# kimerein/sabatinilab-glm

Measured on AMD Instinct MI355X. Metric: IRLS iters/sec on 1M×2000 design mat; CV-grid wall-clock (5-fold×20 λ), lower is better.
Workload: dtype bf16 Hessian (w rounded to bf16, X exact 0/1) / exact-f32 gradient (3 bf16 pieces, f64 slab sums) / f64 coefficients and line search

## Files before the change

### sabatinilab-glm_amd/csrc/lagw.hip

```cpp
#include <algorithm>
#include <cstring>
#include <functional>
#include <map>
#include <mutex>
#include <queue>
#include <type_traits>
#include <vector>

#include "common.h"

namespace sglm {
namespace {

__device__ __forceinline__ int lag_col2(int layout, int m, int K, int b, int ev) {
    return layout ? ev * K + b : b * m + ev;
}

constexpr int kLwRed = 128;

__global__ void __launch_bounds__(256) lag_gram_w_part(const float* __restrict__ W, int64_t ld,
                                                       int32_t n, const int32_t* __restrict__ fits,
                                                       float* __restrict__ part) {
    const float* w = W + (int64_t)fits[blockIdx.y] * ld;
    const int64_t chunk = ((int64_t)n + kLwRed - 1) / kLwRed;
    const int64_t t0 = (int64_t)blockIdx.x * chunk, t1 = min((int64_t)n, t0 + chunk);
    float s = 0.0f;
    for (int64_t t = t0 + threadIdx.x; t < t1; t += 256) s += (float)(__bf16)w[t];
    __shared__ float red[256];
    red[threadIdx.x] = s;
    __syncthreads();
    for (int o = 128; o > 0; o >>= 1) {
        if (threadIdx.x < o) red[threadIdx.x] += red[threadIdx.x + o];
        __syncthreads();
    }
    if (threadIdx.x == 0) part[blockIdx.y * kLwRed + blockIdx.x] = red[0];
}

__global__ void __launch_bounds__(256) lag_gram_w_aux(const float* __restrict__ part,
                                                      const int32_t* __restrict__ fits,
                                                      float* __restrict__ H, int32_t P,
                                                      int32_t p) {
    float* Hf = H + (int64_t)fits[blockIdx.y] * P * P;
    if (blockIdx.x == 0) {
        if (threadIdx.x == 0) {
            float t = 0.0f;
            for (int b = 0; b < kLwRed; ++b) t += part[blockIdx.y * kLwRed + b];
            Hf[(int64_t)p * P + p] = t;
        }
        return;
    }
    const int w = P - p - 1;
    const int64_t tot = (int64_t)P * w;
    for (int64_t e = (int64_t)(blockIdx.x - 1) * 256 + threadIdx.x; e < tot;
         e += (int64_t)(gridDim.x - 1) * 256) {
        const int64_t i = e / w, j = p + 1 + e % w;
        if (i <= j) Hf[i * P + j] = 0.0f;
    }
}

__global__ void __launch_bounds__(256) lag_gram_w_prep(const float* __restrict__ W, int64_t ld,
                                                       int32_t n, const int32_t* __restrict__ fits,
                                                       int32_t nf, int32_t row0, int32_t smin,
                                                       int64_t wlen, int64_t zrow,
                                                       uint16_t* __restrict__ Wt) {
    const int c = blockIdx.y;
    for (int64_t j = (int64_t)blockIdx.x * 256 + threadIdx.x; j < wlen;
         j += (int64_t)gridDim.x * 256) {
        const int64_t i = j + c;
        const int64_t u = i / nf;
        const int f = (int)(i % nf);
        const int64_t t = u - row0 + smin;
        const float x = (t >= 0 && t < n && u < zrow) ? W[(int64_t)fits[f] * ld + t] : 0.0f;
        Wt[c * wlen + j] = __builtin_bit_cast(uint16_t, (__bf16)x);
    }
}

constexpr int kKS2 = 128;
constexpr int kKP2 = kKS2 / 2;
constexpr int kRX2 = kKP2 + 4;
constexpr int kRS2 = 4 * kRX2 + 4;
constexpr int kSentR = -(1 << 28);
constexpr uint32_t kSentW = 0xfffff000u;

typedef short s16x4 __attribute__((ext_vector_type(4)));
typedef __attribute__((address_space(3))) s16x4 lds_s16x4;

struct LagW2Args {
    const uint16_t* Wt;
    int64_t wlen;
    const uint64_t* R;
    const int32_t* occ;
    const int32_t* ev_off;
    const int32_t* bidx;
    const int32_t* fits;
    float* H;
    float* Hb;
    int32_t nf, P, p, m, K, smin, smax, layout, nraw, D, Gm, Gy;
    int32_t njobs;
    int32_t ms;
    int32_t wsh;
    uint16_t jobs[256];
#ifdef SGLM_LAGW_TRACE
    uint64_t* trace;
#endif
};

template <int NCH>
__device__ __forceinline__ int lagw_swz(int row) {
    return NCH == 16 ? ((row & 3) << 2) : (((row >> 1) & 1) << 2);
}

template <int MT, int NT, int WM, int WN, int NH>
struct LagW2Smem {
    static constexpr int MB = WM * MT, NN = WN * NT * 32, ND = MB / NH;
    uint32_t rw[2][ND * kRS2];
    __attribute__((aligned(16))) uint16_t ws[2][kKS2 * NN];
    int32_t vo[4][kKS2];
    uint32_t wo[4][kKS2];
};

template <int MT, int NT, int WM, int WN, int NH>
__global__ void __launch_bounds__(64 * WM * WN) __attribute__((amdgpu_waves_per_eu(2, 2)))
lag_gram_w2_kernel(LagW2Args a) {
    using SM = LagW2Smem<MT, NT, WM, WN, NH>;
    constexpr int NTH = 64 * WM * WN, MB = SM::MB, NN = SM::NN, ND = SM::ND, NCH = NN / 8;
    static_assert(MB % NH == 0, "d rows per piece");
    static_assert((kKS2 * NCH) % NTH == 0, "weight tasks per thread");
    constexpr int kWT = kKS2 * NCH / NTH;
    static_assert((kKP2 * ND) % NTH == 0, "row-word tasks per thread");
    constexpr int kRT = kKP2 * ND / NTH;
    static_assert(kWT <= 4, "staging pieces per K-step");
    __shared__ SM sm;
#ifdef SGLM_LAGW_TRACE
    const uint64_t t_beg = __builtin_amdgcn_s_memrealtime();
#endif
    const int blk = blockIdx.x;
    const int a1 = blk % a.ms;
    if (a1 >= a.m) return;
    int type, half = 0;
    if (a.njobs > 0) {
        if (blk >= a.njobs * a.ms) return;
        const int jb = a.jobs[blk / a.ms];
        type = jb & 0x3fff;
        half = jb >> 14;
    } else {
        type = blk / a.ms;
        if (type >= a.Gm * a.Gy) return;
    }
    const int g = type % a.Gm, y = type / a.Gm;
    const int Tm = a.D * NH;
    const int t0 = g * MB;
    if (t0 >= Tm) return;
    const int di0 = t0 / NH;
    const int n0 = y * NN + a.wsh * di0 * a.nf;
    if (n0 / a.nf >= a.K || min(a.K - 1, (n0 + NN - 1) / a.nf) < di0) return;
    int o_beg = a.ev_off[a1], o_end = a.ev_off[a1 + 1];
    if (half) {
        const int hs = ((o_end - o_beg + kKS2 - 1) / kKS2 + 1) / 2;
        if (half == 1) o_end = min(o_end, o_beg + hs * kKS2);
        else o_beg += hs * kKS2;
    }
    const int nst = max(0, (o_end - o_beg + kKS2 - 1) / kKS2);
    const int tid = threadIdx.x, lane = tid & 63, wave = tid >> 6, h = lane >> 5, r = lane & 31;
    const int wm = wave % WM, wn = wave / WM;

    const __amdgpu_buffer_rsrc_t rsR =
        __builtin_amdgcn_make_buffer_rsrc((void*)a.R, 0, a.nraw * 8, 0x00020000);
    const __amdgpu_buffer_rsrc_t rsW =
        __builtin_amdgcn_make_buffer_rsrc((void*)a.Wt, 0, (int)(uint32_t)(a.wlen * 16), 0x00020000);
    const __amdgpu_buffer_rsrc_t rsO =
        __builtin_amdgcn_make_buffer_rsrc((void*)a.occ, 0, a.ev_off[a.m] * 4, 0x00020000);

    int wk[kWT], wsl[kWT];
#pragma unroll
    for (int i = 0; i < kWT; ++i) {
        const int t = tid + NTH * i;
        wk[i] = t / NCH;
        const int ch = t % NCH;
        wsl[i] = wk[i] * NN + 8 * (ch ^ lagw_swz<NCH>(wk[i]));
        wk[i] = wk[i] | (ch << 16);
    }
    int rkp[kRT], rdl[kRT];
#pragma unroll
    for (int i = 0; i < kRT; ++i) {
        const int t = tid + NTH * i;
        rkp[i] = t / ND;
        rdl[i] = t % ND;
    }

    u32x4 wA[kWT];
    u32x2 rA[kRT][2];
    int32_t oreg = 0;
    bool ovalid = false;

    auto occ_load = [&](int s) __attribute__((always_inline)) {
        const int o = o_beg + s * kKS2 + (tid & (kKS2 - 1));
        ovalid = o < o_end;
        oreg = __builtin_amdgcn_raw_buffer_load_b32(rsO, o * 4, 0, 0);
    };
    auto occ_store = [&](int s) __attribute__((always_inline)) {
        if (tid < kKS2) {
            const int v = ovalid ? oreg : kSentR;
            const int64_t x = (int64_t)(ovalid ? oreg : 0) * a.nf + n0;
            const int c = (int)(x & 7);
            sm.vo[s & 3][tid] = v;
            sm.wo[s & 3][tid] = ovalid ? (uint32_t)(2 * (c * a.wlen + x - c)) : kSentW;
        }
    };
    auto load_w = [&](int s, int i) __attribute__((always_inline)) {
        const uint32_t off = sm.wo[s & 3][wk[i] & 0xffff];
        wA[i] = __builtin_bit_cast(u32x4, __builtin_amdgcn_raw_buffer_load_b128(
                                              rsW, off + 16 * (wk[i] >> 16), 0, 0));
    };
    auto load_r = [&](int s) __attribute__((always_inline)) {
#pragma unroll
        for (int i = 0; i < kRT; ++i)
#pragma unroll
            for (int j = 0; j < 2; ++j) {
                const int u = sm.vo[s & 3][2 * rkp[i] + j] + di0 + rdl[i];
                rA[i][j] = __builtin_bit_cast(
                    u32x2, __builtin_amdgcn_raw_buffer_load_b64(rsR, (uint32_t)u << 3, 0, 0));
            }
    };
    auto store_w = [&](int buf, int i) __attribute__((always_inline)) {
        *reinterpret_cast<u32x4*>(&sm.ws[buf][wsl[i]]) = wA[i];
    };
    auto store_r = [&](int buf) __attribute__((always_inline)) {
#pragma unroll
        for (int i = 0; i < kRT; ++i) {
            uint32_t* dst = &sm.rw[buf][rdl[i] * kRS2 + rkp[i]];
#pragma unroll
            for (int pl = 0; pl < NH; ++pl) {
                const uint32_t w0 = rA[i][0][pl], w1 = rA[i][1][pl];
                dst[(2 * pl) * kRX2] = __builtin_amdgcn_perm(w1, w0, 0x05040100u);
                dst[(2 * pl + 1) * kRX2] = __builtin_amdgcn_perm(w1, w0, 0x07060302u);
            }
        }
    };
    auto data_load = [&](int s) __attribute__((always_inline)) {
#pragma unroll
        for (int i = 0; i < kWT; ++i) load_w(s, i);
        load_r(s);
    };
    auto data_store = [&](int buf) __attribute__((always_inline)) {
#pragma unroll
        for (int i = 0; i < kWT; ++i) store_w(buf, i);
        store_r(buf);
    };

    f32x16 acc[MT][NT];
#pragma unroll
    for (int i = 0; i < MT; ++i)
#pragma unroll
        for (int j = 0; j < NT; ++j) acc[i][j] = (f32x16){};

    int aoff[MT];
    int dmin_w = 1 << 30;
#pragma unroll
    for (int i = 0; i < MT; ++i) {
        const int tau = min(t0 + wm * MT + i, Tm - 1);
        const int dl = tau / NH - di0, hf = tau % NH;
        aoff[i] = dl * kRS2 + (2 * hf + (r >> 4)) * kRX2 + 4 * h;
        if (t0 + wm * MT + i < Tm) dmin_w = min(dmin_w, di0 + dl);
    }
    int j0 = NT, j1 = -1;
#pragma unroll
    for (int j = 0; j < NT; ++j) {
        const int c0 = n0 + (wn * NT + j) * 32;
        const int sb_lo = c0 / a.nf, sb_hi = min(a.K - 1, (c0 + 31) / a.nf);
        if (sb_lo < a.K && sb_hi >= dmin_w) {
            j0 = min(j0, j);
            j1 = max(j1, j);
        }
    }
    const int jcode = __builtin_amdgcn_readfirstlane(j0 > j1 ? -1 : j0 * NT + j1);
    int boff[NT];
    {
        const int g4 = lane >> 4, q = (lane >> 2) & 3, pp = lane & 3;
        const int row = 8 * (g4 >> 1) + q;
#pragma unroll
        for (int j = 0; j < NT; ++j) {
            const int col = (wn * NT + j) * 32 + 16 * (g4 & 1) + 4 * pp;
            boff[j] = row * NN * 2 + 16 * ((col >> 3) ^ lagw_swz<NCH>(row)) + 8 * (pp & 1);
        }
    }
    const uint32_t rsh = (uint32_t)(r - 14 - 16 * (r >> 4)) & 31u;

    auto compute = [&](int s, auto J0c, auto J1c) __attribute__((always_inline)) {
        constexpr int J0 = decltype(J0c)::value, J1 = decltype(J1c)::value;
        const int buf = s & 1;
        const uint32_t* rwb = &sm.rw[buf][0];
        const char* wsb = reinterpret_cast<const char*>(&sm.ws[buf][0]);
        auto fetch = [&](int ks, u32x4 (&wq)[MT], s16x4 (&t1)[NT], s16x4 (&t2)[NT])
                         __attribute__((always_inline)) {
#pragma unroll
            for (int j = J0; j <= J1; ++j) {
                const char* pb = wsb + boff[j] + ks * 16 * NN * 2;
                t1[j] = __builtin_amdgcn_ds_read_tr16_b64_v4i16(
                    (lds_s16x4*)(__attribute__((address_space(3))) char*)pb);
                t2[j] = __builtin_amdgcn_ds_read_tr16_b64_v4i16(
                    (lds_s16x4*)(__attribute__((address_space(3))) char*)(pb + 4 * NN * 2));
            }
#pragma unroll
            for (int i = 0; i < MT; ++i)
                wq[i] = *reinterpret_cast<const u32x4*>(rwb + aoff[i] + 8 * ks);
        };
        auto mult = [&](const u32x4 (&wq)[MT], const s16x4 (&t1)[NT], const s16x4 (&t2)[NT])
                        __attribute__((always_inline)) {
            bf16x8 bq[NT];
#pragma unroll
            for (int j = J0; j <= J1; ++j) {
                const uint2 u1 = __builtin_bit_cast(uint2, t1[j]);
                const uint2 u2 = __builtin_bit_cast(uint2, t2[j]);
                bq[j] = __builtin_bit_cast(bf16x8, make_uint4(u1.x, u1.y, u2.x, u2.y));
            }
            bf16x8 aq[MT];
#pragma unroll
            for (int i = 0; i < MT; ++i) {
                uint32_t dq[4];
#pragma unroll
                for (int q = 0; q < 4; ++q) dq[q] = rotr32(wq[i][q], rsh) & 0x40004000u;
                aq[i] = __builtin_bit_cast(bf16x8, make_uint4(dq[0], dq[1], dq[2], dq[3]));
            }
#pragma unroll
            for (int i = 0; i < MT; ++i)
#pragma unroll
                for (int j = J0; j <= J1; ++j)
                    acc[i][j] = __builtin_amdgcn_mfma_f32_32x32x16_bf16(aq[i], bq[j], acc[i][j],
                                                                        0, 0, 0);
        };
        auto staging = [&](int ks) __attribute__((always_inline)) {
            if (ks < kWT) store_w(buf ^ 1, ks);
            if (ks == kWT) store_r(buf ^ 1);
            if (ks == 4) occ_load(s + 4);
            if (ks >= 4 && ks - 4 < kWT) load_w(s + 2, ks - 4);
            if (ks == 7) load_r(s + 2);
        };
        u32x4 wq[2][MT];
        s16x4 t1[2][NT], t2[2][NT];
        fetch(0, wq[0], t1[0], t2[0]);
#pragma unroll
        for (int ks = 0; ks < kKS2 / 16; ++ks) {
            staging(ks);
            if (ks + 1 < kKS2 / 16)
                fetch(ks + 1, wq[(ks + 1) & 1], t1[(ks + 1) & 1], t2[(ks + 1) & 1]);
            __builtin_amdgcn_sched_barrier(0);
            mult(wq[ks & 1], t1[ks & 1], t2[ks & 1]);
            __builtin_amdgcn_sched_barrier(0);
        }
    };
    auto main_loop = [&](auto J0c, auto J1c) __attribute__((always_inline)) {
#pragma unroll
        for (int j = 0; j < 3; ++j) {
            occ_load(j);
            occ_store(j);
        }
        __syncthreads();
        data_load(0);
        data_store(0);
        occ_load(3);
        data_load(1);
        for (int s = 0; s < nst; ++s) {
            occ_store(s + 3);
            __syncthreads();
            compute(s, J0c, J1c);
        }
    };
    using I0 = std::integral_constant<int, 0>;
    using I1 = std::integral_constant<int, 1>;
    using I2 = std::integral_constant<int, 2>;
    using I3 = std::integral_constant<int, 3>;
    using IN = std::integral_constant<int, -1>;
    if (nst > 0) {
        if constexpr (NT == 4) {
            switch (jcode) {
                case 0: main_loop(I0{}, I0{}); break;
                case 1: main_loop(I0{}, I1{}); break;
                case 2: main_loop(I0{}, I2{}); break;
                case 3: main_loop(I0{}, I3{}); break;
                case 5: main_loop(I1{}, I1{}); break;
                case 6: main_loop(I1{}, I2{}); break;
                case 7: main_loop(I1{}, I3{}); break;
                case 10: main_loop(I2{}, I2{}); break;
                case 11: main_loop(I2{}, I3{}); break;
                case 15: main_loop(I3{}, I3{}); break;
                default: main_loop(I0{}, IN{}); break;
            }
        } else {
            static_assert(NT == 2, "N tiles per wave");
            switch (jcode) {
                case 0: main_loop(I0{}, I0{}); break;
                case 1: main_loop(I0{}, I1{}); break;
                case 3: main_loop(I1{}, I1{}); break;
                default: main_loop(I0{}, IN{}); break;
            }
        }
    }

#pragma unroll
    for (int j = 0; j < NT; ++j) {
        const int nn = n0 + (wn * NT + j) * 32 + r;
        const int sb = nn / a.nf, f = nn % a.nf;
        if (sb >= a.K) continue;
        const int b1 = a.bidx[sb];
        if (b1 < 0) continue;
        float* Hrow = (half == 2 ? a.Hb + (int64_t)f * a.P * a.P
                                 : a.H + (int64_t)a.fits[f] * a.P * a.P) +
                      (int64_t)lag_col2(a.layout, a.m, a.K, b1, a1) * a.P;
#pragma unroll
        for (int i = 0; i < MT; ++i) {
            const int tau = t0 + wm * MT + i;
            if (tau >= Tm) continue;
            const int dd = tau / NH;
            const int hf = tau % NH;
            if (sb < dd) continue;
            const int b2 = a.bidx[sb - dd];
            if (b2 < 0) continue;
#pragma unroll
            for (int q = 0; q < 16; ++q) {
                const int a2 = 32 * hf + (q & 3) + 8 * (q >> 2) + 4 * h;
                const float val = 0.5f * acc[i][j][q];
                if (a2 < a.m) {
                    if (dd == 0 && a2 < a1) continue;
                    Hrow[lag_col2(a.layout, a.m, a.K, b2, a2)] = val;
                } else if (a2 == a.m && dd == 0) {
                    Hrow[a.p] = val;
                }
            }
        }
    }
#ifdef SGLM_LAGW_TRACE
    __syncthreads();
    if (tid == 0) {
        const uint64_t t_end = __builtin_amdgcn_s_memrealtime();
        const uint32_t hw = __builtin_amdgcn_s_getreg(4 | (31 << 11));
        const uint32_t xcc = __builtin_amdgcn_s_getreg(20 | (31 << 11));
        a.trace[4 * blk + 0] = t_beg;
        a.trace[4 * blk + 1] = t_end;
        a.trace[4 * blk + 2] = (uint64_t)hw | ((uint64_t)xcc << 32);
        a.trace[4 * blk + 3] = (uint64_t)type | ((uint64_t)a1 << 16) | ((uint64_t)nst << 32);
    }
#endif
}

struct LagwSplit {
    const float* Hb;
    int32_t smin, nh, MB, NN, Gm, nf, wsh;
    uint32_t mask[8];
};

__global__ void __launch_bounds__(256) lag_gram_w_sym(float* __restrict__ H,
                                                      const int32_t* __restrict__ fits, int32_t P,
                                                      int32_t p, int32_t m, int32_t K,
                                                      int32_t layout,
                                                      const int32_t* __restrict__ shifts,
                                                      LagwSplit sp) {
    __shared__ float tl[64][65], tb[64][65];
    __shared__ int ks_i[64], ks_j[64];
    const int T = P / 64;
    int I = 0, rem = blockIdx.x;
    while (rem >= T - I) { rem -= T - I; ++I; }
    const int J = I + rem;
    float* Hf = H + (int64_t)fits[blockIdx.y] * P * P;
    const float* Hbf = sp.Hb ? sp.Hb + (int64_t)blockIdx.y * P * P : nullptr;
    const int tid = threadIdx.x;
    const int plag = m * K;
    if (tid < 128) {
        const int c = (tid < 64 ? I : J) * 64 + (tid & 63);
        int key = -1;
        if (c < plag) {
            const int b = layout ? c % K : c / m, e = layout ? c / K : c % m;
            key = (shifts[b] + 65536) * 64 + (63 - e);
        }
        (tid < 64 ? ks_i : ks_j)[tid & 63] = key;
    }
    auto split = [&](int kr, int kc, int a2) -> bool {
        if (!Hbf) return false;
        const int s1 = kr / 64 - 65536, s2 = kc / 64 - 65536;
        const int tau = (s1 - s2) * sp.nh + a2 / 32;
        const int g = tau / sp.MB;
        const int y = ((s1 - sp.smin - sp.wsh * (g * sp.MB / sp.nh)) * sp.nf + (int)blockIdx.y) /
                      sp.NN;
        const int t = g + sp.Gm * y;
        return (sp.mask[t >> 5] >> (t & 31)) & 1u;
    };
    for (int e = tid; e < 64 * 64; e += 256) {
        const int rr = e >> 6, cc = e & 63;
        tl[rr][cc] = Hf[(int64_t)(J * 64 + rr) * P + I * 64 + cc];
        if (Hbf) tb[rr][cc] = Hbf[(int64_t)(J * 64 + rr) * P + I * 64 + cc];
    }
    __syncthreads();
    for (int e = tid; e < 64 * 64; e += 256) {
        const int il = e >> 6, jl = e & 63;
        const int i = I * 64 + il, j = J * 64 + jl;
        if (i > j) continue;
        float* dst = Hf + (int64_t)i * P + j;
        if (j > p) {
            *dst = 0.0f;
            continue;
        }
        const int ki = ks_i[il], kj = ks_j[jl];
        if (i == j) {
            if (ki >= 0) {
                if (split(ki, ki, 63 - ki % 64)) *dst += Hbf[(int64_t)i * P + j];
            } else if (i < p) {
                *dst = 0.0f;
            }
            continue;
        }
        if (j == p) {
            if (i >= plag) *dst = 0.0f;
            else if (split(ki, ki, m)) *dst += Hbf[(int64_t)i * P + j];
            continue;
        }
        if (ki < 0 || kj < 0) *dst = 0.0f;
        else if (kj > ki)
            *dst = split(kj, ki, 63 - ki % 64) ? tl[jl][il] + tb[jl][il] : tl[jl][il];
        else if (split(ki, kj, 63 - kj % 64))
            *dst += Hbf[(int64_t)i * P + j];
    }
}

struct LagwPlan {
    int njobs = 0;
    bool split = false;
    uint16_t jobs[256];
    uint32_t mask[8] = {0, 0, 0, 0, 0, 0, 0, 0};
};

static int lagw_cus() {
    static const int n = [] {
        int dev = 0, v = 0;
        if (hipGetDevice(&dev) != hipSuccess ||
            hipDeviceGetAttribute(&v, hipDeviceAttributeMultiprocessorCount, dev) != hipSuccess ||
            v <= 0)
            v = 256;
        return v;
    }();
    return n;
}

static LagwPlan lagw_plan(int m, int K, int nf, int NH, int MT, int NT, int WM, int Gm, int Gy,
                          bool can_split, int wsh) {
    static std::mutex mu;
    static std::map<std::vector<int>, LagwPlan> cache;
    const char* e = getenv("SGLM_LAGW_SPLIT");
    const bool sp_ok = can_split && !(e && e[0] == '0');
    const std::vector<int> key{m, K, nf, NH, MT, NT, WM, Gm, Gy, sp_ok, wsh};
    std::lock_guard<std::mutex> lk(mu);
    auto it = cache.find(key);
    if (it != cache.end()) return it->second;
    LagwPlan pl;
    const int per = Gm * Gy, MB = WM * MT, NN = NT * 32, Tm = K * NH;
    if (per > 128) return cache[key] = pl;
    std::vector<std::pair<double, int>> types;
    for (int t = 0; t < per; ++t) {
        const int g = t % Gm, y = t / Gm;
        const int t0 = g * MB, di0 = t0 / NH, n0 = y * NN + wsh * di0 * nf;
        if (t0 >= Tm || n0 / nf >= K || std::min(K - 1, (n0 + NN - 1) / nf) < di0) continue;
        int simd[4] = {0, 0, 0, 0};
        for (int wm = 0; wm < WM; ++wm) {
            int dmin = 1 << 30;
            for (int i = 0; i < MT; ++i)
                if (t0 + wm * MT + i < Tm) dmin = std::min(dmin, (t0 + wm * MT + i) / NH);
            int j0 = NT, j1 = -1;
            for (int j = 0; j < NT; ++j) {
                const int c0 = n0 + 32 * j;
                if (c0 / nf < K && std::min(K - 1, (c0 + 31) / nf) >= dmin) {
                    j0 = std::min(j0, j);
                    j1 = std::max(j1, j);
                }
            }
            simd[wm % 4] += j1 >= j0 ? MT * (j1 - j0 + 1) : 0;
        }
        const int mx = std::max(std::max(simd[0], simd[1]), std::max(simd[2], simd[3]));
        types.push_back({mx + 7.0, t});
    }
    std::stable_sort(types.begin(), types.end(),
                     [](const std::pair<double, int>& x, const std::pair<double, int>& y) {
                         return x.first > y.first;
                     });
    const int nt = (int)types.size();
    if (nt == 0) {
        pl.njobs = -1;
        return cache[key] = pl;
    }
    const int ncu = lagw_cus();
    const double fix = 0.02 * types[0].first;
    int best_ns = 0;
    double best = 0.0;
    for (int ns = 0; ns <= (sp_ok ? nt : 0); ++ns) {
        if (nt + ns > 256) break;
        std::vector<double> jc;
        for (int i = 0; i < nt; ++i) {
            const double c = types[i].first;
            if (i < ns) jc.insert(jc.end(), 2 * (size_t)m, 0.5 * c + fix);
            else jc.insert(jc.end(), (size_t)m, c);
        }
        std::stable_sort(jc.begin(), jc.end(), std::greater<double>());
        std::priority_queue<double, std::vector<double>, std::greater<double>> q;
        for (int c = 0; c < ncu; ++c) q.push(0.0);
        double mk = 0.0;
        for (double c : jc) {
            const double t = q.top() + c;
            q.pop();
            q.push(t);
            mk = std::max(mk, t);
        }
        if (ns == 0 || mk < best * 0.98) {
            best = mk;
            best_ns = ns;
        }
    }
    std::vector<std::pair<double, int>> jl;
    for (int i = 0; i < nt; ++i) {
        const double c = types[i].first;
        const int t = types[i].second;
        if (i < best_ns) {
            jl.push_back({0.5 * c + fix, t | (1 << 14)});
            jl.push_back({0.5 * c + fix, t | (2 << 14)});
            pl.mask[t >> 5] |= 1u << (t & 31);
        } else {
            jl.push_back({c, t});
        }
    }
    std::stable_sort(jl.begin(), jl.end(),
                     [](const std::pair<double, int>& x, const std::pair<double, int>& y) {
                         return x.first > y.first;
                     });
    pl.njobs = (int)jl.size();
    pl.split = best_ns > 0;
    for (int i = 0; i < pl.njobs; ++i) pl.jobs[i] = (uint16_t)jl[i].second;
    return cache[key] = pl;
}

std::mutex g_tmu;
bool g_ton = false;
std::vector<hipEvent_t> g_tpool;
std::vector<std::pair<hipEvent_t, hipEvent_t>> g_trec;

hipEvent_t lagw_event() {
    if (!g_tpool.empty()) {
        hipEvent_t e = g_tpool.back();
        g_tpool.pop_back();
        return e;
    }
    hipEvent_t e = nullptr;
    return hipEventCreate(&e) == hipSuccess ? e : nullptr;
}

template <int MT, int NT, int WM, int WN, int NH>
int launch_lagw2(const LagW2Args& a0, hipStream_t s, LagwSplit& sp) {
    LagW2Args a = a0;
    constexpr int MB = WM * MT, NN = WN * NT * 32;
    static_assert(WN == 1, "one wave column");
    a.Gm = (a.D * NH + MB - 1) / MB;
    a.Gy = (a.nf * a.K + NN - 1) / NN;
    const char* ew = getenv("SGLM_LAGW_WSHIFT");
    a.wsh = (ew && ew[0] == '0') ? 0 : 1;
    const LagwPlan pl = lagw_plan(a.m, a.K, a.nf, NH, MT, NT, WM, a.Gm, a.Gy, a.Hb != nullptr,
                                  a.wsh);
    if (pl.njobs < 0) return SGLM_OK;
    sp.Hb = pl.split ? a.Hb : nullptr;
    sp.smin = a.smin;
    sp.nh = NH;
    sp.MB = MB;
    sp.NN = NN;
    sp.Gm = a.Gm;
    sp.nf = a.nf;
    sp.wsh = a.wsh;
    std::memcpy(sp.mask, pl.mask, sizeof(sp.mask));
    a.ms = a.m;
    unsigned nblk;
    if (pl.njobs > 0) {
        a.njobs = pl.njobs;
        std::memcpy(a.jobs, pl.jobs, sizeof(a.jobs));
        nblk = (unsigned)(pl.njobs * a.ms);
    } else {
        a.njobs = 0;
        nblk = (unsigned)(a.Gm * a.Gy * a.ms);
    }
#ifdef SGLM_LAGW_TRACE
    hipMalloc(&a.trace, (size_t)nblk * 32);
    hipMemsetAsync(a.trace, 0, (size_t)nblk * 32, s);
#endif
    hipEvent_t t0 = nullptr, t1 = nullptr;
    {
        std::lock_guard<std::mutex> lk(g_tmu);
        if (g_ton) {
            t0 = lagw_event();
            t1 = lagw_event();
        }
    }
    if (t0 && t1) (void)hipEventRecord(t0, s);
    lag_gram_w2_kernel<MT, NT, WM, WN, NH><<<dim3(nblk), 64 * WM * WN, 0, s>>>(a);
    if (t0 && t1) {
        (void)hipEventRecord(t1, s);
        std::lock_guard<std::mutex> lk(g_tmu);
        g_trec.push_back({t0, t1});
    }
#ifdef SGLM_LAGW_TRACE
    {
        static int seq = 0;
        std::vector<uint64_t> tr((size_t)nblk * 4);
        hipStreamSynchronize(s);
        hipMemcpy(tr.data(), a.trace, tr.size() * 8, hipMemcpyDeviceToHost);
        hipFree(a.trace);
        const char* out = getenv("SGLM_LAGW_TRACE_OUT");
        if (out) {
            char path[512];
            snprintf(path, sizeof(path), "%s_%d_nf%d.bin", out, seq++, a.nf);
            if (FILE* f = fopen(path, "wb")) {
                fwrite(tr.data(), 8, tr.size(), f);
                fclose(f);
            }
        }
    }
#endif
    return check_launch("lag_gram_w2_kernel");
}

}
}

using namespace sglm;

static int64_t lagw_zrow(int32_t nraw, int32_t K) { return (int64_t)nraw + K + 8; }
static int64_t lagw_wlen(int32_t nraw, int32_t K, int32_t nf) {
    return ((lagw_zrow(nraw, K) + K + 8) * nf + 512 + 7) / 8 * 8;
}

static size_t lagw_hb_off(int32_t nraw, int32_t K, int32_t nf) {
    return ((size_t)(8 * lagw_wlen(nraw, K, nf) * 2) + (size_t)nf * kLwRed * 4 + 255) / 256 * 256;
}

extern "C" size_t sglm_lag_gram_w_work_bytes(int32_t nraw, int32_t K, int32_t nf, int32_t P) {
    return lagw_hb_off(nraw, K, nf) + (size_t)nf * P * P * 4;
}

extern "C" int sglm_lag_gram_w(const uint64_t* R, const int32_t* occ, const int32_t* ev_off,
                               int32_t m, int32_t nraw, const int32_t* shifts,
                               const int32_t* bidx, int32_t K, int32_t smin, int32_t smax,
                               int32_t layout, int32_t row0, int32_t n, const float* W,
                               int64_t ld, const int32_t* fits, int32_t nf, float* H, int32_t P,
                               int32_t pones, void* work, sglm_stream_t stream) {
    if (nf <= 0) return SGLM_OK;
    const int p = pones;
    if (!R || !occ || !ev_off || !shifts || !bidx || !W || !fits || !H || !work || m < 1 ||
        m > 63 || K < 1 || smax - smin + 1 != K || p < K * m || p + 1 > P || n < 0 || ld < n) {
        set_error("sglm_lag_gram_w: bad args (m=%d K=%d P=%d)", m, K, P);
        return SGLM_EINVAL;
    }
    const int64_t wlen = lagw_wlen(nraw, K, nf);
    if (nraw >= (1 << 28) || wlen >= ((int64_t)1 << 27)) {
        set_error("sglm_lag_gram_w: %d raw rows x %d fits exceed one launch (split the fits)",
                  nraw, nf);
        return SGLM_EINVAL;
    }
    hipStream_t s = as_stream(stream);
    LagW2Args b{};
    b.wlen = wlen;
    b.Wt = (const uint16_t*)work;
    lag_gram_w_prep<<<dim3(1024, 8), 256, 0, s>>>(W, ld, n, fits, nf, row0, smin, b.wlen,
                                                  lagw_zrow(nraw, K), (uint16_t*)work);
    {
        const int st0 = check_launch("lag_gram_w_prep");
        if (st0) return st0;
    }
    b.R = R; b.occ = occ; b.ev_off = ev_off; b.bidx = bidx;
    b.fits = fits; b.H = H; b.nf = nf; b.P = P; b.p = p; b.m = m; b.K = K;
    b.smin = smin; b.smax = smax; b.layout = layout; b.nraw = nraw;
    b.D = K;
    float* part = (float*)((uint16_t*)work + 8 * b.wlen);
    lag_gram_w_part<<<dim3(kLwRed, (unsigned)nf), 256, 0, s>>>(W, ld, n, fits, part);
    b.Hb = (float*)((char*)work + lagw_hb_off(nraw, K, nf));
    const bool two = m + 1 > 32;
    LagwSplit sp{};
    const int st = (nf * K <= 64) ? (two ? launch_lagw2<2, 2, 8, 1, 2>(b, s, sp)
                                         : launch_lagw2<2, 2, 8, 1, 1>(b, s, sp))
                                  : (two ? launch_lagw2<2, 4, 8, 1, 2>(b, s, sp)
                                         : launch_lagw2<2, 4, 8, 1, 1>(b, s, sp));
    if (st) return st;
    const int T = P / 64;
    lag_gram_w_sym<<<dim3((unsigned)(T * (T + 1) / 2), (unsigned)nf), 256, 0, s>>>(
        H, fits, P, p, m, K, layout, shifts, sp);
    lag_gram_w_aux<<<dim3(1, (unsigned)nf), 256, 0, s>>>(part, fits, H, P, p);
    return check_launch("lag_gram_w_aux");
}

extern "C" int sglm_lag_gram_w_timing(int32_t mode, double* ms, int32_t* n) {
    std::lock_guard<std::mutex> lk(g_tmu);
    if (mode == 0) {
        g_ton = false;
        return SGLM_OK;
    }
    double tot = 0.0;
    int cnt = 0;
    for (auto& pr : g_trec) {
        if (mode == 2) {
            float x = 0.0f;
            if (hipEventSynchronize(pr.second) == hipSuccess &&
                hipEventElapsedTime(&x, pr.first, pr.second) == hipSuccess) {
                tot += x;
                ++cnt;
            }
        }
        g_tpool.push_back(pr.first);
        g_tpool.push_back(pr.second);
    }
    g_trec.clear();
    if (mode == 1) g_ton = true;
    if (ms) *ms = tot;
    if (n) *n = cnt;
    return SGLM_OK;
}

__global__ void __launch_bounds__(256) lag_rowwords_kernel(const int32_t* __restrict__ ebits,
                                                           int32_t m, int32_t nwords,
                                                           int32_t nraw, uint64_t* __restrict__ R) {
    const int u = blockIdx.x * 256 + threadIdx.x;
    if (u >= nraw) return;
    uint64_t x = (uint64_t)1 << m;
    for (int e = 0; e < m; ++e)
        x |= (uint64_t)(((uint32_t)ebits[(int64_t)e * nwords + (u >> 5)] >> (u & 31)) & 1u) << e;
    R[u] = x;
}

extern "C" int sglm_lag_rowwords(const int32_t* ebits, int32_t m, int32_t nwords, int32_t nraw,
                                 uint64_t* R, sglm_stream_t stream) {
    if (!ebits || !R || m < 1 || m > 63 || nraw < 0 || nwords * 32 < nraw) {
        set_error("sglm_lag_rowwords: bad args");
        return SGLM_EINVAL;
    }
    if (nraw == 0) return SGLM_OK;
    lag_rowwords_kernel<<<(nraw + 255) / 256, 256, 0, as_stream(stream)>>>(ebits, m, nwords, nraw,
                                                                           R);
    return check_launch("lag_rowwords_kernel");
}
```

Measured before the change: 0.02516.

## Fuse lag-Gram weight prep with partial sums, cut shifted copies to two

The bf16 weight staging kernel now writes only two shifted copies instead of eight. Each thread converts a run of eight values and stores them with 16-byte vector writes, and the main kernel's copy selection and buffer bound change to match. The diagonal partial-sum reduction is folded into the prep launch as extra blocks, and the aux kernel's final sum is moved into the symmetrize kernel. This removes two launches and most of the staging traffic, and the split lookup uses shifts instead of divisions. The risks are correctness of the two-copy alignment scheme and the dropped zeroing of the H entries beyond the ones column, which the old aux kernel performed.

```diff
diff --git a/sabatinilab-glm_amd/csrc/lagw.hip b/sabatinilab-glm_amd/csrc/lagw.hip
--- a/sabatinilab-glm_amd/csrc/lagw.hip
+++ b/sabatinilab-glm_amd/csrc/lagw.hip
@@ -17,62 +17,54 @@
 }
 
 constexpr int kLwRed = 128;
-
-__global__ void __launch_bounds__(256) lag_gram_w_part(const float* __restrict__ W, int64_t ld,
-                                                       int32_t n, const int32_t* __restrict__ fits,
-                                                       float* __restrict__ part) {
-    const float* w = W + (int64_t)fits[blockIdx.y] * ld;
-    const int64_t chunk = ((int64_t)n + kLwRed - 1) / kLwRed;
-    const int64_t t0 = (int64_t)blockIdx.x * chunk, t1 = min((int64_t)n, t0 + chunk);
-    float s = 0.0f;
-    for (int64_t t = t0 + threadIdx.x; t < t1; t += 256) s += (float)(__bf16)w[t];
-    __shared__ float red[256];
-    red[threadIdx.x] = s;
-    __syncthreads();
-    for (int o = 128; o > 0; o >>= 1) {
-        if (threadIdx.x < o) red[threadIdx.x] += red[threadIdx.x + o];
-        __syncthreads();
-    }
-    if (threadIdx.x == 0) part[blockIdx.y * kLwRed + blockIdx.x] = red[0];
-}
-
-__global__ void __launch_bounds__(256) lag_gram_w_aux(const float* __restrict__ part,
-                                                      const int32_t* __restrict__ fits,
-                                                      float* __restrict__ H, int32_t P,
-                                                      int32_t p) {
-    float* Hf = H + (int64_t)fits[blockIdx.y] * P * P;
-    if (blockIdx.x == 0) {
-        if (threadIdx.x == 0) {
-            float t = 0.0f;
-            for (int b = 0; b < kLwRed; ++b) t += part[blockIdx.y * kLwRed + b];
-            Hf[(int64_t)p * P + p] = t;
-        }
-        return;
-    }
-    const int w = P - p - 1;
-    const int64_t tot = (int64_t)P * w;
-    for (int64_t e = (int64_t)(blockIdx.x - 1) * 256 + threadIdx.x; e < tot;
-         e += (int64_t)(gridDim.x - 1) * 256) {
-        const int64_t i = e / w, j = p + 1 + e % w;
-        if (i <= j) Hf[i * P + j] = 0.0f;
-    }
-}
+constexpr int kLwCopies = 2;
 
 __global__ void __launch_bounds__(256) lag_gram_w_prep(const float* __restrict__ W, int64_t ld,
                                                        int32_t n, const int32_t* __restrict__ fits,
                                                        int32_t nf, int32_t row0, int32_t smin,
                                                        int64_t wlen, int64_t zrow,
-                                                       uint16_t* __restrict__ Wt) {
-    const int c = blockIdx.y;
-    for (int64_t j = (int64_t)blockIdx.x * 256 + threadIdx.x; j < wlen;
-         j += (int64_t)gridDim.x * 256) {
-        const int64_t i = j + c;
-        const int64_t u = i / nf;
-        const int f = (int)(i % nf);
+                                                       uint16_t* __restrict__ Wt, int32_t nprep,
+                                                       float* __restrict__ part) {
+    if ((int)blockIdx.x >= nprep) {
+        const int pb = blockIdx.x - nprep, q = pb / kLwRed, b = pb % kLwRed;
+        const float* w = W + (int64_t)fits[q] * ld;
+        const int64_t chunk = ((int64_t)n + kLwRed - 1) / kLwRed;
+        const int64_t t0 = (int64_t)b * chunk, t1 = min((int64_t)n, t0 + chunk);
+        float s = 0.0f;
+        for (int64_t t = t0 + threadIdx.x; t < t1; t += 256) s += (float)(__bf16)w[t];
+        __shared__ float red[256];
+        red[threadIdx.x] = s;
+        __syncthreads();
+        for (int o = 128; o > 0; o >>= 1) {
+            if (threadIdx.x < o) red[threadIdx.x] += red[threadIdx.x + o];
+            __syncthreads();
+        }
+        if (threadIdx.x == 0) part[pb] = red[0];
+        return;
+    }
+    const int64_t i0 = ((int64_t)blockIdx.x * 256 + threadIdx.x) * 8;
+    if (i0 >= wlen) return;
+    int64_t u = i0 / nf;
+    int f = (int)(i0 % nf);
+    uint32_t x[9];
+#pragma unroll
+    for (int e = 0; e < 9; ++e) {
         const int64_t t = u - row0 + smin;
-        const float x = (t >= 0 && t < n && u < zrow) ? W[(int64_t)fits[f] * ld + t] : 0.0f;
-        Wt[c * wlen + j] = __builtin_bit_cast(uint16_t, (__bf16)x);
-    }
+        const float v = (t >= 0 && t < n && u < zrow) ? W[(int64_t)fits[f] * ld + t] : 0.0f;
+        x[e] = __builtin_bit_cast(uint16_t, (__bf16)v);
+        if (++f == nf) {
+            f = 0;
+            ++u;
+        }
+    }
+    u32x4 c0, c1;
+#pragma unroll
+    for (int q = 0; q < 4; ++q) {
+        c0[q] = x[2 * q] | (x[2 * q + 1] << 16);
+        c1[q] = x[2 * q + 1] | (x[2 * q + 2] << 16);
+    }
+    *reinterpret_cast<u32x4*>(Wt + i0) = c0;
+    *reinterpret_cast<u32x4*>(Wt + wlen + i0) = c1;
 }
 
 constexpr int kKS2 = 128;
@@ -167,7 +159,8 @@
     const __amdgpu_buffer_rsrc_t rsR =
         __builtin_amdgcn_make_buffer_rsrc((void*)a.R, 0, a.nraw * 8, 0x00020000);
     const __amdgpu_buffer_rsrc_t rsW =
-        __builtin_amdgcn_make_buffer_rsrc((void*)a.Wt, 0, (int)(uint32_t)(a.wlen * 16), 0x00020000);
+        __builtin_amdgcn_make_buffer_rsrc((void*)a.Wt, 0, (int)(uint32_t)(a.wlen * 2 * kLwCopies),
+                                          0x00020000);
     const __amdgpu_buffer_rsrc_t rsO =
         __builtin_amdgcn_make_buffer_rsrc((void*)a.occ, 0, a.ev_off[a.m] * 4, 0x00020000);
 
@@ -202,7 +195,7 @@
         if (tid < kKS2) {
             const int v = ovalid ? oreg : kSentR;
             const int64_t x = (int64_t)(ovalid ? oreg : 0) * a.nf + n0;
-            const int c = (int)(x & 7);
+            const int c = (int)(x & (kLwCopies - 1));
             sm.vo[s & 3][tid] = v;
             sm.wo[s & 3][tid] = ovalid ? (uint32_t)(2 * (c * a.wlen + x - c)) : kSentW;
         }
@@ -445,7 +438,7 @@
 
 struct LagwSplit {
     const float* Hb;
-    int32_t smin, nh, MB, NN, Gm, nf, wsh;
+    int32_t smin, nh_sh, MB_sh, NN_sh, Gm, nf, wsh;
     uint32_t mask[8];
 };
 
@@ -454,6 +447,7 @@
                                                       int32_t p, int32_t m, int32_t K,
                                                       int32_t layout,
                                                       const int32_t* __restrict__ shifts,
+                                                      const float* __restrict__ part,
                                                       LagwSplit sp) {
     __shared__ float tl[64][65], tb[64][65];
     __shared__ int ks_i[64], ks_j[64];
@@ -474,14 +468,19 @@
         }
         (tid < 64 ? ks_i : ks_j)[tid & 63] = key;
     }
+    if (blockIdx.x == 0 && tid == 255) {
+        float t = 0.0f;
+        for (int b = 0; b < kLwRed; ++b) t += part[blockIdx.y * kLwRed + b];
+        Hf[(int64_t)p * P + p] = t;
+    }
     auto split = [&](int kr, int kc, int a2) -> bool {
         if (!Hbf) return false;
         const int s1 = kr / 64 - 65536, s2 = kc / 64 - 65536;
-        const int tau = (s1 - s2) * sp.nh + a2 / 32;
-        const int g = tau / sp.MB;
-        const int y = ((s1 - sp.smin - sp.wsh * (g * sp.MB / sp.nh)) * sp.nf + (int)blockIdx.y) /
-                      sp.NN;
-        const int t = g + sp.Gm * y;
+        const int tau = ((s1 - s2) << sp.nh_sh) + (a2 >> 5);
+        const int g = tau >> sp.MB_sh;
+        const int di0 = (g << sp.MB_sh) >> sp.nh_sh;
+        const int y = ((s1 - sp.smin - sp.wsh * di0) * sp.nf + (int)blockIdx.y) >> sp.NN_sh;
+        const int t = (g + sp.Gm * y) & 255;
         return (sp.mask[t >> 5] >> (t & 31)) & 1u;
     };
     for (int e = tid; e < 64 * 64; e += 256) {
@@ -663,9 +662,11 @@
     if (pl.njobs < 0) return SGLM_OK;
     sp.Hb = pl.split ? a.Hb : nullptr;
     sp.smin = a.smin;
-    sp.nh = NH;
-    sp.MB = MB;
-    sp.NN = NN;
+    static_assert((NH & (NH - 1)) == 0 && (MB & (MB - 1)) == 0 && (NN & (NN - 1)) == 0,
+                  "LagwSplit's shift counts");
+    sp.nh_sh = __builtin_ctz(NH);
+    sp.MB_sh = __builtin_ctz(MB);
+    sp.NN_sh = __builtin_ctz(NN);
     sp.Gm = a.Gm;
     sp.nf = a.nf;
     sp.wsh = a.wsh;
@@ -731,7 +732,8 @@
 }
 
 static size_t lagw_hb_off(int32_t nraw, int32_t K, int32_t nf) {
-    return ((size_t)(8 * lagw_wlen(nraw, K, nf) * 2) + (size_t)nf * kLwRed * 4 + 255) / 256 * 256;
+    return ((size_t)(kLwCopies * lagw_wlen(nraw, K, nf) * 2) + (size_t)nf * kLwRed * 4 + 255) /
+           256 * 256;
 }
 
 extern "C" size_t sglm_lag_gram_w_work_bytes(int32_t nraw, int32_t K, int32_t nf, int32_t P) {
@@ -747,7 +749,8 @@
     if (nf <= 0) return SGLM_OK;
     const int p = pones;
     if (!R || !occ || !ev_off || !shifts || !bidx || !W || !fits || !H || !work || m < 1 ||
-        m > 63 || K < 1 || smax - smin + 1 != K || p < K * m || p + 1 > P || n < 0 || ld < n) {
+        m > 63 || K < 1 || smax - smin + 1 != K || p < K * m || p + 1 > P || n < 0 || ld < n ||
+        ((uintptr_t)work & 15)) {
         set_error("sglm_lag_gram_w: bad args (m=%d K=%d P=%d)", m, K, P);
         return SGLM_EINVAL;
     }
@@ -761,8 +764,10 @@
     LagW2Args b{};
     b.wlen = wlen;
     b.Wt = (const uint16_t*)work;
-    lag_gram_w_prep<<<dim3(1024, 8), 256, 0, s>>>(W, ld, n, fits, nf, row0, smin, b.wlen,
-                                                  lagw_zrow(nraw, K), (uint16_t*)work);
+    float* part = (float*)((uint16_t*)work + kLwCopies * b.wlen);
+    const int nprep = (int)((b.wlen / 8 + 255) / 256);
+    lag_gram_w_prep<<<dim3((unsigned)(nprep + nf * kLwRed)), 256, 0, s>>>(
+        W, ld, n, fits, nf, row0, smin, b.wlen, lagw_zrow(nraw, K), (uint16_t*)work, nprep, part);
     {
         const int st0 = check_launch("lag_gram_w_prep");
         if (st0) return st0;
@@ -771,8 +776,6 @@
     b.fits = fits; b.H = H; b.nf = nf; b.P = P; b.p = p; b.m = m; b.K = K;
     b.smin = smin; b.smax = smax; b.layout = layout; b.nraw = nraw;
     b.D = K;
-    float* part = (float*)((uint16_t*)work + 8 * b.wlen);
-    lag_gram_w_part<<<dim3(kLwRed, (unsigned)nf), 256, 0, s>>>(W, ld, n, fits, part);
     b.Hb = (float*)((char*)work + lagw_hb_off(nraw, K, nf));
     const bool two = m + 1 > 32;
     LagwSplit sp{};
@@ -783,9 +786,8 @@
     if (st) return st;
     const int T = P / 64;
     lag_gram_w_sym<<<dim3((unsigned)(T * (T + 1) / 2), (unsigned)nf), 256, 0, s>>>(
-        H, fits, P, p, m, K, layout, shifts, sp);
-    lag_gram_w_aux<<<dim3(1, (unsigned)nf), 256, 0, s>>>(part, fits, H, P, p);
-    return check_launch("lag_gram_w_aux");
+        H, fits, P, p, m, K, layout, shifts, part, sp);
+    return check_launch("lag_gram_w_sym");
 }
 
 extern "C" int sglm_lag_gram_w_timing(int32_t mode, double* ms, int32_t* n) {
```

Result: no change. 0.02533, median of 2 (+0.7%).
